# Healthcare-Robotics/assistive-vr-gym

Measured on AMD Instinct MI355X. Metric: env-steps/sec at N parallel envs, 1/2/4/8 MI355X; max |dq| vs PyBullet, higher is better.
Workload: dtype f32; 1 GPU; FeedingJaco-v0, 4096 envs/GPU, rigid-only, random actions; task=FeedingJaco-v0, envs_per_gpu=4096, impairment=random, parallelism=env-sharded x1, env_groups=4, stepping=rollout

## Files before the change

assistive-vr-gym_amd/csrc/avr_kernel.hip:

```cpp
#include <hip/hip_runtime.h>
#include <stdint.h>

#include "../../include/avr.h"
#include <cstring>
#include <cstdlib>
#include "avr_math.h"

#include "avr_kmodel.h"

typedef float f2v __attribute__((ext_vector_type(2)));
typedef float f4v __attribute__((ext_vector_type(4)));
typedef __attribute__((address_space(3))) float lds_f;
#define AVR_GA __attribute__((address_space(1)))
template <class T> __device__ __forceinline__ T gld(const T *p) { return *(const AVR_GA T *)p; }
__device__ __forceinline__ int2 gld(const int2 *p) { const AVR_GA int *q = (const AVR_GA int *)p; return make_int2(q[0], q[1]); }
__device__ __forceinline__ float2 gld(const float2 *p) { const f2v x = *(const AVR_GA f2v *)p; return make_float2(x.x, x.y); }
__device__ __forceinline__ float4 gld(const float4 *p) { const f4v x = *(const AVR_GA f4v *)p; return make_float4(x.x, x.y, x.z, x.w); }
__device__ __forceinline__ v3 gld3(const float *p) { const AVR_GA float *q = (const AVR_GA float *)p; return V(q[0], q[1], q[2]); }
__device__ __forceinline__ qt gldq(const float *p) { const AVR_GA float *q = (const AVR_GA float *)p; return Q(q[0], q[1], q[2], q[3]); }
__device__ __forceinline__ tf gldtf(const float *p) { tf r; r.p = gld3(p); r.q = gldq(p + 3); return r; }
typedef __attribute__((address_space(3))) f2v lds_f2;
typedef __attribute__((address_space(3))) f4v lds_f4;
typedef __attribute__((address_space(3))) int lds_i;
typedef const __attribute__((address_space(1))) float *gfp;
// ... 3380 lines not shown
        pcount(36, sm);
        pcount(37, mx);
        pcount(38, __popcll(__ballot(pk == 3)));
        pcount(39, __popcll(__ballot(pk >= 0 && pk < 3)));
#endif
    }
}

__global__ __launch_bounds__(64) __attribute__((amdgpu_waves_per_eu(NP_WAVES))) void avr_narrowphase_kernel(const KModel *__restrict__ mp, const float *__restrict__ state,
                                                             const unsigned char *__restrict__ mask, int env0, int n_envs) {
    const int list = (blockIdx.x >> 3) & 1;
    const int eb = env0 + 8 * NP_ENVS * (blockIdx.x >> 4) + (blockIdx.x & 7);
    if (eb >= n_envs) return;
    __shared__ float2 ent[NP_ENVS * MAXSP];
    __shared__ float btfs[NP_ENVS][MAXB * 8];
    __shared__ __attribute__((aligned(16))) int hkey[NP_HOT_KEYS];
    np_list(*mp, state, mask, eb, list, n_envs, ent, btfs, hkey);
}

#ifndef AVR_COOP_KERNEL
#define AVR_COOP_KERNEL 0
#endif
#if AVR_COOP_KERNEL
__global__ __launch_bounds__(64) void avr_coop_kernel(const KModel *__restrict__ mp, const unsigned char *__restrict__ mask, int env0, int n_envs) {
    __shared__ EpaBuf E;
    AVR_ENV_GUARD();
    if (gld(env_cs(m, env) + CS_COOP) != 0.f) {
        float *ws = env_ws(m, env);
        const int rot = __float_as_int(gld(ws + WS_COOPROT));
        (void)np_coop(m, env_cs(m, env), __float_as_int(gld(env_cs(m, env) + CS_NSP)), E, rot, 1 << 30);
        if (lane_id() == 0) ws[WS_COOPROT] = __int_as_float(rot + AVR_COOP_CAP);
    }
}
#endif

AVR_DI void substep_a_env(const KModel &m, EnvLDS &L, float *__restrict__ state, float dt, int env, int n_envs) {
    (void)n_envs;
    WT_START();
    static_assert(sizeof(EpaBuf) <= sizeof(EnvLDS), "EPA buffer overlay");
#if !AVR_COOP_KERNEL
    float *gst = state + (size_t)env * K_STATE_WORDS;
    const bool persist = gld(gst + S_TASK + T_COOPN) >= (float)AVR_COOP_PERSIST;
    int demand = 0;
    if (gld(env_cs(m, env) + CS_COOP) != 0.f) {
        float *ws = env_ws(m, env);
        const int rot = __float_as_int(gld(ws + WS_COOPROT));
        demand = np_coop(m, env_cs(m, env), __float_as_int(gld(env_cs(m, env) + CS_NSP)), *reinterpret_cast<EpaBuf *>(&L), rot,
                         persist ? AVR_COOP_CAP : 1 << 30);
        if (lane_id() == 0) ws[WS_COOPROT] = __int_as_float(rot + AVR_COOP_CAP);
        SYNC();
    }
#endif
#if AVR_COOP_KERNEL
    float *gst = state + (size_t)env * K_STATE_WORDS;
#endif
    load_a(m, L, gst, env_cs(m, env));
#if !AVR_COOP_KERNEL
    if (lane_id() == 0) {
        L.st[S_TASK + T_COOPN] = demand > AVR_COOP_CAP ? L.st[S_TASK + T_COOPN] + 1.f : 0.f;
        if (persist && demand > AVR_COOP_CAP) L.flags |= 32;
    }
    SYNC();
#endif
    bool ok = substep_a(m, L, dt, gst, env_ws(m, env), env_rows(m, env), env_cs(m, env), K_DYN_ROLE ? env_dynho(m, env) : nullptr);
#ifdef AVR_PROF
    if (lane_id() == 0) env_ws(m, env)[WS_XCC] = __int_as_float(xcc_id());
#endif
    if (lane_id() == 0 && !ok) L.flags |= 1;
    SYNC();
    if (lane_id() == 0) L.st[S_TASK + T_FLAGS] = (float)((int)L.st[S_TASK + T_FLAGS] | L.flags);
    SYNC();
    if (lane_id() < 16) gst[S_TASK + lane_id()] = L.st[S_TASK + lane_id()];
    prof_flush(m, L, env);
    WT_END(0);
}

__global__ __launch_bounds__(64) AVR_KATTR void avr_substep_a_kernel(const KModel *__restrict__ mp, float *__restrict__ state,
                                                                     const unsigned char *__restrict__ mask, float dt, int env0, int n_envs) {
    __shared__ EnvLDS L;
    AVR_ENV_GUARD();
    substep_a_env(m, L, state, dt, env, n_envs);
}

#if B4_PK
struct DV { float rq, rq2; f2v v1, v2, v3; };
#else
struct DV { float rq, rq2, vx, vy, vz, wx, wy, wz; };
#endif

AVR_DI int uni(int x) { return __builtin_amdgcn_readfirstlane(x); }

#define B4_OOB 0x7fff0000
typedef __amdgpu_buffer_rsrc_t rsrc_t;
typedef unsigned u4v __attribute__((ext_vector_type(4)));
typedef unsigned u3v __attribute__((ext_vector_type(3)));
typedef unsigned u2v __attribute__((ext_vector_type(2)));
AVR_DI f4v bld4(rsrc_t r, int o) { u4v x = __builtin_amdgcn_raw_buffer_load_b128(r, o, 0, 0); return *(f4v *)&x; }
AVR_DI f2v bld2(rsrc_t r, int o) { u2v x = __builtin_amdgcn_raw_buffer_load_b64(r, o, 0, 0); return *(f2v *)&x; }
AVR_DI float bld1(rsrc_t r, int o) { return __uint_as_float(__builtin_amdgcn_raw_buffer_load_b32(r, o, 0, 0)); }
#if NDL == 2
typedef f4v rv_t;
#define RVB 16
#define rload bld4
#else
typedef f2v rv_t;
#define RVB 8
#define rload bld2
#endif
typedef __attribute__((address_space(3))) rv_t lds_rv;
AVR_DI f4v bld3(rsrc_t r, int o) {
    u3v x = __builtin_amdgcn_raw_buffer_load_b96(r, o, 0, 0);
    f4v y = {__uint_as_float(x.x), __uint_as_float(x.y), __uint_as_float(x.z), 0.f};
    return y;
}

#ifndef B4_LDSW
#define B4_LDSW 10240
#endif
AVR_DI int al4(int x) { return (x + 3) & ~3; }

#ifndef B4_ADDR
#define B4_ADDR 1
#endif
#define B4_NP (B4_ADDR && B4_NC_LDS ? 1 : 0)
AVR_DI unsigned lds_addr(const __attribute__((address_space(3))) void *p) { return (unsigned)(size_t)p; }
AVR_DI __attribute__((address_space(3))) float *lds_at(unsigned a) { return (__attribute__((address_space(3))) float *)(size_t)a; }

AVR_DI int own_of(int mask) {
    const int sl = lane_id() & 15;
    return (int)__builtin_amdgcn_ubfe((unsigned)mask, sl < MAXF ? 2 * sl : 30, 2);
}
static_assert(2 * MAXF <= CI_SLOT && MAXNC + K_CROWS * K_MAX_CONTACTS < (1 << (30 - CI_SLOT)), "own mask and slot bit fields");


struct NcRow { int o; lds_f *ip; f4v h0, h1; float imp; f2v j0, j1, j2; rv_t r; };
struct NcSrc {
    typedef NcRow Row;
    static constexpr bool robot_parts = true, addr = false;
    rsrc_t rs;
    int eo, ro;
    lds_f *ip0, *nullip;
    AVR_DI void set(Row &R, bool v, int o, lds_f *ip) const { R.o = v ? o : B4_OOB; R.ip = v ? ip : nullip; }
    AVR_DI void hdr(Row &R) const { R.h0 = bld4(rs, R.o); R.h1 = bld3(rs, R.o + 16); R.imp = *R.ip; }
    AVR_DI void parts(Row &R) const {
        const int o = own_of(__float_as_int(R.h0.x));
        const int b = o ? R.o + 8 + 24 * o : B4_OOB;
        R.j0 = bld2(rs, b); R.j1 = bld2(rs, b + 8); R.j2 = bld2(rs, b + 16);
        const int slot = __float_as_int(R.h0.y) - 1;
        R.r = rload(rs, slot >= 0 ? ro + slot * (ROBW * 4) + RVB * (lane_id() & 15) : B4_OOB);
    }
};

#define LN_HEAD (NDL == 2 ? 80 : 48)
#define LNB_NULL 24
#define LNB_ZERO 48
#define LNB_NCNULL 16
typedef __attribute__((address_space(3))) char lds_c;
struct NcLds {
    typedef NcRow Row;
    static constexpr bool robot_parts = true, addr = B4_ADDR != 0;
    lds_c *blk;
    int eo;
    unsigned rob;
    lds_f *ip0, *nullip;
    AVR_DI void set(Row &R, bool v, int o, lds_f *ip) const { R.o = v ? o : LNB_NCNULL; R.ip = v ? ip : nullip; }
    AVR_DI void hdr(Row &R) const {
        R.h0 = *(const lds_f4 *)(blk + R.o - 8);
        const f2v a = *(const lds_f2 *)(blk + R.o + 8);
        R.h1.x = a.x; R.h1.y = a.y; R.h1.z = *(const lds_f *)(blk + R.o + 16);
        R.imp = *R.ip;
    }
    AVR_DI void parts(Row &R) const {
        const int w = own_of(__float_as_int(R.h0.x));
        const lds_f2 *q = (const lds_f2 *)(blk + (w ? R.o + 24 * w : LNB_ZERO));
        R.j0 = q[0]; R.j1 = q[1]; R.j2 = q[2];
        const unsigned sp = (unsigned)__float_as_int(R.h0.y);
        R.r = *(const lds_rv *)(blk + (sp ? rob + ROBW * 4 * sp : LNB_ZERO));
    }
};

struct CRowL { unsigned wb; lds_f *ip; f4v h; float imp; f2v j0, j1, j2; rv_t r; };
template <bool RC>
struct CLds {
    typedef CRowL Row;
    static constexpr bool robot_parts = RC, addr = B4_ADDR != 0;
    lds_c *blk;
    unsigned cn, cf;
    unsigned rob;
    lds_f *ipn, *ipf, *nullip;
    unsigned ct;
    lds_f *ipt;
    AVR_DI void set(Row &R, bool v, unsigned wb, lds_f *ip) const { R.wb = v ? wb : LNB_NULL; R.ip = v ? ip : nullip; }
    AVR_DI void hdr(Row &R) const { R.h = *(const lds_f4 *)(blk + R.wb + 8); R.imp = *R.ip; }
    AVR_DI void hdr3(Row &R) const {
        const lds_f *q = (const lds_f *)(blk + R.wb + 8);
        const f2v a = *(const lds_f2 *)q;
        R.h.x = a.x; R.h.y = a.y; R.h.z = q[2];
        R.imp = *R.ip;
    }
    AVR_DI void hdr2(Row &B, const Row &A) const {
        B.h = *(const lds_f4 *)(blk + A.wb + 8 + CRW * 4);
        B.imp = A.ip[1];
    }
    AVR_DI unsigned own_b(const Row &R) const { const int o = own_of(__float_as_int(R.h.x)); return o ? R.wb + 24 * o : LNB_ZERO; }
    AVR_DI void own_at(Row &R, unsigned b) const { const lds_f2 *q = (const lds_f2 *)(blk + b); R.j0 = q[0]; R.j1 = q[1]; R.j2 = q[2]; }
    AVR_DI unsigned rob_b(const Row &R) const { const unsigned s = (unsigned)__float_as_int(R.h.x) >> CI_SLOT; return s ? rob + ROBW * 4 * s : LNB_ZERO; }
    AVR_DI rv_t rob_at(unsigned b) const {
// ... 49 lines not shown
#pragma clang fp contract(off)
#if B4_PK
    f2v s = X.j0 * d.v1;
    if (RP) {
        s.y = fmaf(X.r.x, d.rq, s.y);
#if NDL == 2
        s.y = fmaf(X.r.z, d.rq2, s.y);
#endif
    }
    s = __builtin_elementwise_fma(X.j1, d.v2, s);
    s = __builtin_elementwise_fma(X.j2, d.v3, s);
    const float dv = row16_sum(s.x + s.y);
    const float ni = __builtin_amdgcn_fmed3f(imp + fmaf(-dv, inv, rhs), lo, hi);
    const float delta = ni - imp;
    if (acc) *acc |= __ballot(fabsf(delta) > rl);
    const f2v dd = {delta, delta};
    d.v1 = __builtin_elementwise_fma(X.j0, dd, d.v1);
    d.v2 = __builtin_elementwise_fma(X.j1, dd, d.v2);
    d.v3 = __builtin_elementwise_fma(X.j2, dd, d.v3);
    if (RP) d.rq = fmaf(X.r.y, delta, d.rq);
#if NDL == 2
    if (RP) d.rq2 = fmaf(X.r.w, delta, d.rq2);
#endif
    return ni;
#else
    const float p = fmaf(X.j1.x, d.vz, fmaf(X.j0.y, d.vy, X.j0.x * d.vx));
#if NDL == 2
    const float q = RP ? fmaf(X.j2.y, d.wz, fmaf(X.j2.x, d.wy, fmaf(X.r.z, d.rq2, fmaf(X.r.x, d.rq, X.j1.y * d.wx))))
                       : fmaf(X.j2.y, d.wz, fmaf(X.j2.x, d.wy, X.j1.y * d.wx));
#else
    const float q = RP ? fmaf(X.j2.y, d.wz, fmaf(X.j2.x, d.wy, fmaf(X.r.x, d.rq, X.j1.y * d.wx)))
                       : fmaf(X.j2.y, d.wz, fmaf(X.j2.x, d.wy, X.j1.y * d.wx));
#endif
    const float dv = row16_sum(p + q);
    const float ni = __builtin_amdgcn_fmed3f(imp + fmaf(-dv, inv, rhs), lo, hi);
    const float delta = ni - imp;
    if (acc) *acc |= __ballot(fabsf(delta) > rl);
    d.vx = fmaf(X.j0.x, delta, d.vx); d.vy = fmaf(X.j0.y, delta, d.vy); d.vz = fmaf(X.j1.x, delta, d.vz);
    d.wx = fmaf(X.j1.y, delta, d.wx); d.wy = fmaf(X.j2.x, delta, d.wy); d.wz = fmaf(X.j2.y, delta, d.wz);
    if (RP) d.rq = fmaf(X.r.y, delta, d.rq);
#if NDL == 2
    if (RP) d.rq2 = fmaf(X.r.w, delta, d.rq2);
#endif
    return ni;
#endif
}

#if B4_FPAIR
template <bool RP, class R>
AVR_DI void go4_pair(const R &A, const R &B, DV &d, float &ia, float &ib, float lim) {
#pragma clang fp contract(off)
    f2v sa = A.j0 * d.v1, sb = B.j0 * d.v1;
    if (RP) {
        sa.y = fmaf(A.r.x, d.rq, sa.y); sb.y = fmaf(B.r.x, d.rq, sb.y);
#if NDL == 2
        sa.y = fmaf(A.r.z, d.rq2, sa.y); sb.y = fmaf(B.r.z, d.rq2, sb.y);
#endif
    }
    sa = __builtin_elementwise_fma(A.j1, d.v2, sa); sb = __builtin_elementwise_fma(B.j1, d.v2, sb);
    sa = __builtin_elementwise_fma(A.j2, d.v3, sa); sb = __builtin_elementwise_fma(B.j2, d.v3, sb);
    const float dva = row16_sum(sa.x + sa.y), dvb0 = row16_sum(sb.x + sb.y);
    const float na = __builtin_amdgcn_fmed3f(ia + fmaf(-dva, A.h.y, A.h.z), -lim, lim);
    const float da = na - ia;
    const float dvb = fmaf(da, B.h.w, dvb0);
    const float nb = __builtin_amdgcn_fmed3f(ib + fmaf(-dvb, B.h.y, B.h.z), -lim, lim);
    const float db = nb - ib;
    const f2v dda = {da, da}, ddb = {db, db};
    d.v1 = __builtin_elementwise_fma(B.j0, ddb, __builtin_elementwise_fma(A.j0, dda, d.v1));
    d.v2 = __builtin_elementwise_fma(B.j1, ddb, __builtin_elementwise_fma(A.j1, dda, d.v2));
    d.v3 = __builtin_elementwise_fma(B.j2, ddb, __builtin_elementwise_fma(A.j2, dda, d.v3));
    if (RP) d.rq = fmaf(B.r.y, db, fmaf(A.r.y, da, d.rq));
#if NDL == 2
    if (RP) d.rq2 = fmaf(B.r.w, db, fmaf(A.r.w, da, d.rq2));
#endif
    ia = na; ib = nb;
}
#endif

template <int D, bool H3, class S>
AVR_DI void hdr_of(const S &s, typename S::Row &R) {
    if constexpr (H3) s.hdr3(R);
    else s.hdr(R);
}
template <int D, bool H3, class S, class AT, class GO>
AVR_DI void sweep4(const S &s, int n, const AT &at, const GO &go) {
    if (n <= 0) return;
    constexpr int K = 2 * D + 1;
    typename S::Row R[K];
#pragma unroll
    for (int q = 0; q < 2 * D; q++) { at(R[q], q); hdr_of<D, H3>(s, R[q]); }
#pragma unroll
    for (int q = 0; q < D; q++) s.parts(R[q]);
    for (int j = 0; j < n; j += K) {
#pragma unroll
        for (int q = 0; q < K; q++) {
            at(R[(q + 2 * D) % K], j + q + 2 * D);
            hdr_of<D, H3>(s, R[(q + 2 * D) % K]);
            s.parts(R[(q + D) % K]);
            go(R[q]);
        }
    }
}

template <class S>
struct Pair4 { typename S::Row a, b; float in; };

#if K_TORSION
template <class CS>
struct TorRow : CS::Row { float in; };
template <class CS>
struct TorSrc {
    typedef TorRow<CS> Row;
    static constexpr bool robot_parts = CS::robot_parts;
    const CS &cs;
    AVR_DI void hdr(Row &R) const { cs.hdr(R); }
    AVR_DI void parts(Row &R) const { cs.parts(R); }
};
#endif

AVR_DI int wave_max4(int x) {
    x = max(x, __shfl_xor(x, 16));
    x = max(x, __shfl_xor(x, 32));
    return uni(x);
}

template <int DN, int DC, class NS, class CS>
AVR_DI int pgs4(const KModel &m, const NS &ns, const CS &cs, lds_i *list, lds_i *tlist, int n_nc, int n_c, int nnc_max, int nc_max, DV &d) {
    typedef typename NS::Row NR;
    typedef typename CS::Row CR;
    const int sl = lane_id() & 15;
#if B4_PK
    d.rq = d.rq2 = 0.f; d.v1 = d.v2 = d.v3 = f2v{0.f, 0.f};
#else
    d.rq = d.rq2 = 0.f; d.vx = d.vy = d.vz = d.wx = d.wy = d.wz = 0.f;
#endif
    auto at_n = [&](CR &R, int j) {
        if constexpr (CS::addr) {
            const unsigned k = (unsigned)min(j, n_c);
            R.wb = cs.cn + CRW * 4 * k;
            R.ip = (lds_f *)((lds_c *)cs.ipn + __umul24(k, 12u));
        } else cs.set(R, j < n_c, cs.cn + CRW * 4 * j, cs.ipn + j);
    };
    sweep4<DC, true>(cs, nc_max, at_n, [&](const CR &R) { (void)go4<CS::robot_parts>(R, d, 0.f, R.h.y, R.h.z, R.imp, R.imp); });
    int units = 0;
    bool done = false;
    for (int it = 0; it < m.iters; it++) {
        const int a_nc = done ? 0 : n_nc, a_c = done ? 0 : n_c;
        const int anc_max = wave_max4(a_nc), ac_max = wave_max4(a_c);
        unsigned long long acc = 0ull;
        const bool fwd = (it & 1) != 0;
        const int r0 = fwd ? 0 : n_nc - 1, sg = fwd ? 1 : -1;
        const int ob = ns.eo + r0 * (RWC * 4);
        lds_f *ib = ns.ip0 + r0;
        const int no = fwd ? n_nc - a_nc : a_nc - 1;
        sweep4<DN, false>(ns, anc_max, [&](NR &R, int j) {
                              if constexpr (NS::addr) {
                                  const unsigned k = min((unsigned)(no + sg * j), (unsigned)n_nc);
                                  R.o = ns.eo + (int)__umul24(k, (unsigned)(RWC * 4));
                                  R.ip = ns.ip0 + k;
                              } else ns.set(R, j < a_nc, ob + sg * j * (RWC * 4), ib + sg * j);
                          },
                          [&](const NR &R) { *R.ip = go4<true>(R, d, R.imp, R.h0.z, R.h0.w, R.h1.x, R.h1.y, R.h1.z, &acc); });
        unsigned nb = cs.cn + CRW * 4 * (n_c - a_c);
        lds_c *const nib = (lds_c *)cs.ipn + 12 * (n_c - a_c);
        if constexpr (CS::addr) asm("" : "+v"(nb));
        auto at_na = [&](CR &R, int j) {
            if constexpr (CS::addr) {
                const unsigned k = (unsigned)min(j, a_c);
                R.wb = nb + CRW * 4 * k;
                R.ip = (lds_f *)(nib + __umul24(k, 12u));
            } else cs.set(R, j < a_c, cs.cn + CRW * 4 * j, cs.ipn + j);
        };
        sweep4<DC, false>(cs, ac_max, at_na, [&](const CR &R) { *R.ip = go4<CS::robot_parts>(R, d, R.imp, R.h.y, R.h.z, 0.f, 1e10f, R.h.w, &acc); });
        int t = 0;
        for (int c0 = 0; c0 < ac_max; c0 += 16) {
            const int c = c0 + sl;
            const bool a = c < a_c && cs.ipn[(CS::addr ? 3 : 1) * (c < a_c ? c : 0)] > 0.f;
            const unsigned long long b = __ballot(a);
            const unsigned gm = (unsigned)(b >> (lane_id() & 48)) & 0xffffu;
            if constexpr (CS::addr) {
                if (a) list[t + __popc(gm & ((1u << sl) - 1u))] = (int)((cs.cf + 2 * CRW * 4 * c) | lds_addr(cs.ipf + 3 * c) << 16);
            } else if (a) list[t + __popc(gm & ((1u << sl) - 1u))] = c;
            t += __popc(gm);
        }
        if constexpr (CS::addr) list[t] = (int)((unsigned)LNB_NULL | lds_addr(cs.nullip) << 16);
        const int tmax = wave_max4(t);
        units += tmax;
        if (tmax > 0) {
        constexpr int K = 2 * DC + 1;
        Pair4<CS> X[K];
        auto lst = [&](int u) {
            if constexpr (CS::addr) return list[min(u, t)];
            else { const int c = list[u < t ? u : 0]; return u < t ? c : -1; }
        };
        auto hdr = [&](Pair4<CS> &Y, int c) {
            if constexpr (CS::addr) {
                Y.a.wb = (unsigned)c & 0xffffu;
                Y.a.ip = lds_at((unsigned)c >> 16);
                cs.hdr(Y.a);
                cs.hdr2(Y.b, Y.a);
                Y.in = Y.a.ip[2];
            } else {
                cs.set(Y.a, c >= 0, cs.cf + 2 * CRW * 4 * c, cs.ipf + 2 * c);
                cs.hdr(Y.a);
                cs.hdr2(Y.b, Y.a);
                const float x = cs.ipn[max(c, 0)];
                Y.in = c >= 0 ? x : 0.f;
            }
        };
        auto go = [&](const Pair4<CS> &Y) {
            const float lim = Y.a.h.w * Y.in;
#if B4_FPAIR
            float ia = Y.a.imp, ib = Y.b.imp;
            go4_pair<CS::robot_parts>(Y.a, Y.b, d, ia, ib, lim);
            Y.a.ip[0] = ia; Y.a.ip[1] = ib;
#else
            Y.a.ip[0] = go4<CS::robot_parts>(Y.a, d, Y.a.imp, Y.a.h.y, Y.a.h.z, -lim, lim, Y.b.h.x, &acc);
            Y.a.ip[1] = go4<CS::robot_parts>(Y.b, d, Y.b.imp, Y.b.h.y, Y.b.h.z, -lim, lim, Y.b.h.w, &acc);
#endif
        };
        int cn = lst(0);
#pragma unroll
        for (int q = 0; q < 2 * DC; q++) { hdr(X[q], cn); cn = lst(q + 1); }
#pragma unroll
        for (int q = 0; q < DC; q++) cs.unit_parts(X[q].a, X[q].b);
        for (int u0 = 0; u0 < tmax; u0 += K) {
#pragma unroll
            for (int q = 0; q < K; q++) {
                hdr(X[(q + 2 * DC) % K], cn);
                cn = lst(u0 + q + 2 * DC + 1);
                cs.unit_parts(X[(q + DC) % K].a, X[(q + DC) % K].b);
                go(X[q]);
            }
        }
#if K_TORSION
        if constexpr (CS::addr) {
            typedef __attribute__((address_space(3))) u2v lds_u2;
            lds_u2 *const tl = (lds_u2 *)tlist;
            int tt = 0;
            for (int u0 = 0; u0 < tmax; u0 += 16) {
                const int u = u0 + sl;
                const unsigned e = (unsigned)list[min(u, t)];
                const int c = u < t ? (int)((e & 0xffffu) - cs.cf) >> 7 : 0;
                const int tv = cs.tor_of(c);
                const float in = lds_at(e >> 16)[2];
                const bool a = u < t && tv > 0;
                const unsigned long long b = __ballot(a);
                const unsigned gm = (unsigned)(b >> (lane_id() & 48)) & 0xffffu;
                if (a) {
                    lds_u2 *const q = tl + 3 * (tt + __popc(gm & ((1u << sl) - 1u)));
                    const unsigned w = (cs.ct + 3 * CRW * 4 * (tv - 1)) | lds_addr(cs.ipt + 3 * (tv - 1)) << 16;
#pragma unroll
                    for (int k = 0; k < 3; k++) q[k] = u2v{w + k * (CRW * 4 + (4 << 16)), (unsigned)__float_as_int(in)};
                }
                tt += __popc(gm);
            }
            const int tr = 3 * tt;
            tl[tr] = u2v{(unsigned)LNB_NULL | lds_addr(cs.nullip) << 16, 0u};
            const int ttmax = wave_max4(tt);
            const TorSrc<CS> ts{cs};
            sweep4<DC, false>(ts, 3 * ttmax, [&](TorRow<CS> &R, int j) {
                const u2v e = tl[min(j, tr)];
                R.wb = e.x & 0xffffu;
                R.ip = lds_at(e.x >> 16);
                R.in = __uint_as_float(e.y);
            }, [&](const TorRow<CS> &R) {
                const float lim = R.h.w * R.in;
                *R.ip = go4<CS::robot_parts>(R, d, R.imp, R.h.y, R.h.z, -lim, lim, BT_RESIDUAL_SQRT * R.h.y, &acc);
            });
        } else {
            int tt = 0;
            for (int u0 = 0; u0 < tmax; u0 += 16) {
                const int u = u0 + sl;
                const int cl = list[u < t ? u : 0];
                const int c = u < t ? cl : 0;
                const int tv = cs.tor_of(c);
                const bool a = u < t && tv > 0;
                const unsigned long long b = __ballot(a);
                const unsigned gm = (unsigned)(b >> (lane_id() & 48)) & 0xffffu;
                if (a) tlist[tt + __popc(gm & ((1u << sl) - 1u))] = c | (tv - 1) << 8;
                tt += __popc(gm);
            }
            int ttmax = tt;
            ttmax = max(ttmax, __shfl_xor(ttmax, 16));
            ttmax = max(ttmax, __shfl_xor(ttmax, 32));
            ttmax = uni(ttmax);
            const TorSrc<CS> ts{cs};
            sweep4<DC, false>(ts, 3 * ttmax, [&](TorRow<CS> &R, int j) {
                const int u = j / 3, k = j - 3 * u;
                const bool v = u < tt;
                const int e = tlist[v ? u : 0];
                const int c = e & 255, ti = e >> 8;
                cs.set(R, v, cs.ct + 3 * CRW * 4 * ti + CRW * 4 * k, cs.ipt + 3 * ti + k);
                const float x = cs.ipn[v ? c : 0];
                R.in = v ? x : 0.f;
            }, [&](const TorRow<CS> &R) {
                const float lim = R.h.w * R.in;
                *R.ip = go4<CS::robot_parts>(R, d, R.imp, R.h.y, R.h.z, -lim, lim, BT_RESIDUAL_SQRT * R.h.y, &acc);
            });
        }
#endif
        }
        done = done || ((acc >> (lane_id() & 48)) & 0xffffull) == 0ull;
        if (__ballot(!done) == 0ull) break;
    }
    return units;
}

#ifndef B4_DN
#define B4_DN 2
#endif
#ifndef B4_DC
#define B4_DC 1
#endif
#ifndef B4_DG
#define B4_DG 3
#endif
#ifndef B4_NC_LDS
#define B4_NC_LDS K_PR2
#endif
#ifndef B4_DNL
#define B4_DNL 1
#endif

#ifndef B4_SORT
#define B4_SORT 0
#endif
AVR_DI int b4_env(const KModel &m, const unsigned char *__restrict__ mask, int env0, int n_envs, int bidx, int g) {
    const int x = bidx & 7, j = bidx >> 3;
#if B4_SORT
    const int lane = lane_id();
    const int kc = (j >> 5) << 7;
    unsigned key[2];
#pragma unroll
    for (int h = 0; h < 2; h++) {
        const int kk = lane + 64 * h;
        const int e = env0 + x + 8 * (kc + kk);
        unsigned cost = 0xffffffu;
        if (e < n_envs) {
            cost = 0u;
            if (!mask || mask[e]) {
                const float *ws = env_ws(m, e);
                cost = (unsigned)(__float_as_int(gld(ws + WS_NNC)) + 3 * __float_as_int(gld(ws + WS_NC)) +
                                  (K_TORSION ? 3 * __float_as_int(gld(ws + WS_NT)) : 0));
                cost = min(cost, 0xfffffeu);
            }
        }
        key[h] = (cost << 7) | (unsigned)kk;
    }
    int rank0 = 0, rank1 = 0;
    for (int i = 0; i < 64; i++) {
        const unsigned a = __builtin_amdgcn_readlane(key[0], i), b = __builtin_amdgcn_readlane(key[1], i);
        rank0 += (a < key[0]) + (b < key[0]);
        rank1 += (a < key[1]) + (b < key[1]);
    }
    int pick = 0;
#pragma unroll
    for (int gg = 0; gg < 4; gg++) {
        const int r = 4 * (j & 31) + gg;
        const unsigned long long b0 = __ballot(rank0 == r), b1 = __ballot(rank1 == r);
        const int kk = b0 ? __builtin_ctzll(b0) : 64 + __builtin_ctzll(b1);
        if (g == gg) pick = kk;
    }
    return env0 + x + 8 * (kc + pick);
#else
    (void)m; (void)mask; (void)n_envs;
    return env0 + 32 * j + x + 8 * g;
#endif
}

AVR_DI void substep_b4_block(const KModel &m, float *__restrict__ state, const unsigned char *__restrict__ mask, float dt, int frame_end,
                             int env0, int n_envs, int bidx, lds_f *blk) {
#ifdef AVR_WAVETIME
    const unsigned long long wt0 = __builtin_amdgcn_s_memrealtime();
#endif
    const int lane = lane_id(), sl = lane & 15, g = lane >> 4;
    const int env = b4_env(m, mask, env0, n_envs, bidx, g);
    const bool live = env < n_envs && (!mask || mask[env]);
    const int ev = live ? env : env0;
    const gfp wsg = (gfp)env_ws(m, ev);
    float *st = state + (size_t)ev * K_STATE_WORDS;
    const int n_nc = live ? __float_as_int(wsg[WS_NNC]) : 0, n_c = live ? __float_as_int(wsg[WS_NC]) : 0;
    const int n_rob = live ? __float_as_int(wsg[WS_NROB]) : 0;
    const int n_t = live && K_TORSION ? __float_as_int(wsg[WS_NT]) : 0;
    const int n_cr = 3 * n_c + 3 * n_t;
    const int n_rows = n_nc + n_cr, n_rc = max(n_rob - n_nc, 0);
    auto wmax = [&](int x) { x = max(x, __shfl_xor(x, 16)); x = max(x, __shfl_xor(x, 32)); return uni(x); };
// ... 3 lines not shown
#ifdef AVR_LDS_POISON
    for (int i = lane; i < B4_LDSW; i += 64) blk[i] = __int_as_float(-1);
    SYNC();
#endif
#if B4_ADDR
    constexpr int GN = 4, GNC = 8;
    const int n_imp = n_rows + 3 + B4_NP;
    const int szA = al4(n_imp) + al4(n_c + 1) + (K_TORSION ? al4(6 * n_t + 2) : 0), szB = n_cr * CRW + n_rc * ROBW + GN;
#else
    constexpr int GN = 0, GNC = 0;
    const int n_imp = n_rows + 2;
    const int szA = al4(n_imp) + (K_TORSION ? 2 : 1) * al4(n_c), szB = n_cr * CRW + n_rc * ROBW;
#endif
#if B4_NC_LDS
    const int szF = szB + n_nc * (RWC + ROBW) + GNC;
    const int f0 = __shfl(szA + szF, 0), f1 = __shfl(szA + szF, 16), f2 = __shfl(szA + szF, 32), f3 = __shfl(szA + szF, 48);
    const bool full = uni(f0 + f1 + f2 + f3) <= B4_LDSW - LN_HEAD && !m.b4_global;
#else
    const int f0 = 0, f1 = 0, f2 = 0;
    constexpr bool full = false;
#endif
    const int t0 = __shfl(szA + szB, 0), t1 = __shfl(szA + szB, 16), t2 = __shfl(szA + szB, 32), t3 = __shfl(szA + szB, 48);
    const bool in_lds = full || (uni(t0 + t1 + t2 + t3) <= B4_LDSW - LN_HEAD && !m.b4_global);
    int base;
    if (full) base = g == 0 ? 0 : g == 1 ? f0 : g == 2 ? f0 + f1 : f0 + f1 + f2;
    else if (in_lds) base = g == 0 ? 0 : g == 1 ? t0 : g == 2 ? t0 + t1 : t0 + t1 + t2;
    else {
        const int a0 = __shfl(szA, 0), a1 = __shfl(szA, 16), a2 = __shfl(szA, 32);
        base = g == 0 ? 0 : g == 1 ? a0 : g == 2 ? a0 + a1 : a0 + a1 + a2;
    }
    base += LN_HEAD;
    lds_f *imp = blk + base;
    lds_i *list = (lds_i *)(imp + al4(n_imp));
    lds_i *tlist = list + al4(n_c + (B4_ADDR ? 1 : 0));
    const int cw = base + szA, nw = cw + n_cr * CRW + GN, rw = full ? nw + n_nc * RWC + GNC : nw;
    const bool trip = B4_ADDR && in_lds;
    const int ins = trip ? 3 : 1;
    lds_f *const ipt = trip ? imp + n_nc + B4_NP : imp + n_nc + 3 * n_c;
    lds_f *const ipf = trip ? ipt + 3 * n_t : imp + n_nc + n_c;
    lds_f *const ipn = trip ? ipf + 2 : imp + n_nc;
    lds_f *const nullip = trip ? ipf + 3 * n_c : imp + n_rows;
    const gfp cpool = (gfp)(st + S_CP);
    float wimp[K_MAX_CONTACTS / 16];
#pragma unroll
    for (int q = 0; q < K_MAX_CONTACTS / 16; q++) wimp[q] = cpool[AVR_CP_WORDS * min(sl + 16 * q, max(n_c - 1, 0)) + AVR_CP_IMP];
    for (int r = sl; r < n_imp; r += 16) {
        const int c = r - (int)(ipn - imp);
        if (!(c >= 0 && c < ins * n_c && (!trip || c % 3 == 0))) imp[r] = 0.f;
    }
    for (int i = lane; i < LN_HEAD; i += 64) blk[i] = 0.f;
    if (in_lds) {
        const int n4r = n_cr * (CRW / 4), n4n = full ? n_nc * (RWC / 4) : 0, n4s = (full ? n_rob : n_rc) * (ROBW / 4);
        const int n4a = n4r + n4n, n4 = n4a + n4s, so = full ? ro : ro + n_nc * ROBW * 4;
        const int m4 = wmax(n4);
        lds_f4 *l0 = (lds_f4 *)(blk + cw);
        for (int b = 0; b < m4; b += 8 * 16) {
            f4v t[8];
#pragma unroll
            for (int q = 0; q < 8; q++) {
                const int i = b + 16 * q + sl;
                t[q] = bld4(rs, i < n4r ? eo + CR_BASE * 4 + 16 * i : i < n4a ? eo + 16 * (i - n4r) : (i < n4 ? so + 16 * (i - n4a) : B4_OOB));
            }
#pragma unroll
            for (int q = 0; q < 8; q++) {
                const int i = b + 16 * q + sl;
#if B4_ADDR
                if (i < n4) l0[i + (i >= 4 * n_c ? GN / 4 : 0) + (full && i >= n4a ? GNC / 4 : 0)] = t[q];
#else
                if (i < n4) l0[i] = t[q];
#endif
            }
        }
#if B4_ADDR
        if (sl == 0) l0[4 * n_c] = f4v{0.f, 0.f, 0.f, 0.f};
        if (full && sl < GNC / 4) l0[n4a + GN / 4 + sl] = f4v{0.f, 0.f, 0.f, 0.f};
#endif
    }
#pragma unroll
    for (int q = 0; q < K_MAX_CONTACTS / 16; q++)
        if (sl + 16 * q < n_c) ipn[ins * (sl + 16 * q)] = wimp[q] * m.warmstart;
    SYNC();
    NcSrc ns{rs, eo, ro, imp, nullip};
    DV d;
    int units, rcb = 0;
#if B4_NC_LDS
    if (full) {
        const unsigned cn = 4 * cw - 8, cf = cn + 4 * CRW * n_c + 4 * GN, ct = cf + 8 * CRW * n_c, rob = 4 * (rw - ROBW) + RVB * sl;
        const NcLds nl{(lds_c *)blk, 4 * nw + 8, rob, imp, nullip};
        if (wmax(n_rc) > 0) {
            CLds<true> cs{(lds_c *)blk, cn, cf, rob, ipn, ipf, nullip, ct, ipt};
            units = pgs4<B4_DNL, B4_DC>(m, nl, cs, list, tlist, n_nc, n_c, nnc_max, nc_max, d);
            rcb = 1;
        } else {
            CLds<false> cs{(lds_c *)blk, cn, cf, rob, ipn, ipf, nullip, ct, ipt};
            units = pgs4<B4_DNL, B4_DC>(m, nl, cs, list, tlist, n_nc, n_c, nnc_max, nc_max, d);
        }
    } else
#endif
    if (in_lds) {
        const unsigned cn = 4 * cw - 8, cf = cn + 4 * CRW * n_c + 4 * GN, ct = cf + 8 * CRW * n_c, rob = 4 * (rw - (n_nc + 1) * ROBW) + RVB * sl;
        if (wmax(n_rc) > 0) {
            CLds<true> cs{(lds_c *)blk, cn, cf, rob, ipn, ipf, nullip, ct, ipt};
            units = pgs4<B4_DN, B4_DC>(m, ns, cs, list, tlist, n_nc, n_c, nnc_max, nc_max, d);
            rcb = 1;
        } else {
            CLds<false> cs{(lds_c *)blk, cn, cf, rob, ipn, ipf, nullip, ct, ipt};
            units = pgs4<B4_DN, B4_DC>(m, ns, cs, list, tlist, n_nc, n_c, nnc_max, nc_max, d);
        }
    } else {
        const int cn = eo + CR_BASE * 4, cf = cn + 4 * CRW * n_c, ct = cf + 8 * CRW * n_c, rob = ro - ROBW * 4 + RVB * sl;
        CGlb cs{rs, cn, cf, rob, ipn, ipf, nullip, ct, ipt};
        units = pgs4<B4_DN, B4_DG>(m, ns, cs, list, tlist, n_nc, n_c, nnc_max, nc_max, d);
    }
    (void)units; (void)rcb;
    for (int c = sl; c < n_c; c += 16) st[S_CP + AVR_CP_WORDS * c + AVR_CP_IMP] = ipn[ins * c];
#ifdef AVR_WAVETIME
    {
        const unsigned long long wt1 = __builtin_amdgcn_s_memrealtime();
        const int e0 = env0 + 32 * (bidx >> 3) + (bidx & 7);
        if (m.prof && lane == 0 && e0 < n_envs) {
            m.prof[((size_t)1 * n_envs + e0) * 2] = wt0;
            m.prof[((size_t)1 * n_envs + e0) * 2 + 1] = wt1;
            m.prof[((size_t)2 * n_envs + e0) * 2] = (unsigned long long)nnc_max | (unsigned long long)nc_max << 16 | (unsigned long long)in_lds << 32;
            m.prof[((size_t)2 * n_envs + e0) * 2 + 1] = (unsigned long long)wmax(n_rows) | (unsigned long long)units << 16 | (unsigned long long)rcb << 40 | (unsigned long long)xcc_id() << 44;
        }
    }
#endif
    if (!live) return;
    const float *ws = env_ws(m, ev);
#if B4_PK
    struct { float vx, vy, vz, wx, wy, wz; } dl = {d.v1.x, d.v2.x, d.v3.x, d.v1.y, d.v2.y, d.v3.y};
#else
    DV &dl = d;
#endif
    if (sl < m.nf) {
        const qt q = ldq(st + S_FREE + AVR_FB_WORDS * sl + 3);
        const v3 I = gld3(m.fb_inertia + 4 * sl);
        const float rs = 1.f / sqrtf(gld(m.fb_mass + (sl)));
        const v3 sd = V(sqrtf(I.x > 0.f ? 1.f / I.x : 0.f), sqrtf(I.y > 0.f ? 1.f / I.y : 0.f), sqrtf(I.z > 0.f ? 1.f / I.z : 0.f));
        const v3 w = qrot(q, V(dl.wx * sd.x, dl.wy * sd.y, dl.wz * sd.z));
        dl.vx *= rs; dl.vy *= rs; dl.vz *= rs;
        dl.wx = w.x; dl.wy = w.y; dl.wz = w.z;
    }
    const float vmax = m.max_vel;
    const int nda = env_hdyn(m, st) ? m.nd + m.hc_n : m.nd;
#pragma unroll
    for (int k = 0; k < NDL; k++) {
        const int dof = sl + 16 * k;
        if (dof < nda) {
            float v = clampf(ws[WS_VQ + dof] + (k == 0 ? d.rq : d.rq2), -vmax, vmax);
            float q = st[S_Q + dof] + dt * v;
            if (frame_end && dof >= m.nd) {
#if K_CHAIN_LIMITS_IN_STATE
                const float lo = st[S_HCH + 2 * K_HC_N + (dof - m.nd)], hi = st[S_HCH + 3 * K_HC_N + (dof - m.nd)];
#else
                const float lo = gld(m.hc_lower + (dof - m.nd)), hi = gld(m.hc_upper + (dof - m.nd));
#endif
                if (q < lo) { q = lo; v = 0.f; }
                else if (q > hi) { q = hi; v = 0.f; }
            }
            st[S_QD + dof] = v;
            st[S_Q + dof] = q;
        }
    }
    if (sl < m.nf) {
        float *fb = st + S_FREE + AVR_FB_WORDS * sl;
        v3 v = clamp3(add(ld3(ws + WS_FV + 4 * sl), V(dl.vx, dl.vy, dl.vz)), vmax);
        v3 om = clamp3(add(ld3(ws + WS_FW + 4 * sl), V(dl.wx, dl.wy, dl.wz)), vmax);
        st3(fb + 7, v);
        st3(fb + 10, om);
        st3(fb, add(ld3(fb), scl(v, dt)));
        float ang = len(om);
        if (ang * dt > BT_ANGULAR_MOTION_THRESHOLD) ang = (0.5f * 1.5707963267948966f) / dt;
        v3 ax;
        if (ang < 0.001f) ax = scl(om, 0.5f * dt - (dt * dt * dt) * 0.020833333333f * ang * ang);
        else ax = scl(om, sinf(0.5f * ang * dt) / ang);
        qt dq = Q(ax.x, ax.y, ax.z, cosf(ang * dt * 0.5f));
        stq(fb + 3, qnorm(qmul(dq, ldq(fb + 3))));
    }
}

__global__ __launch_bounds__(64) void avr_substep_b4_kernel(const KModel *__restrict__ mp, float *__restrict__ state,
                                                            const unsigned char *__restrict__ mask, float dt, int frame_end, int env0,
                                                            int n_envs) {
    __shared__ f4v b4l[B4_LDSW / 4];
    substep_b4_block(*mp, state, mask, dt, frame_end, env0, n_envs, blockIdx.x, (lds_f *)(lds_f4 *)b4l);
}



#if AVR_TASK == AVR_TASK_FEEDING
__global__ __launch_bounds__(64) void avr_task_kernel(const KModel *__restrict__ mp, float *__restrict__ state, float *__restrict__ obs,
                                                      float *__restrict__ rew, unsigned char *__restrict__ done, float *__restrict__ info,
                                                      const unsigned char *__restrict__ mask, int mode, int env0, int n_envs) {
    __shared__ EnvLDS L;
    AVR_ENV_GUARD();
    const int lane = lane_id();
    float *gst = state + (size_t)env * K_STATE_WORDS;
    const float *gcp = gst + S_CP;
    load_state(m, L, gst);
    PROF_START(ptask);
    if (L.nla > m.nl) robot_fk(m, L);
    mouth_target(m, L);
    if (mode == MODE_SETTLE) {
        if (obs) observe(m, L, 0.f, obs + (size_t)env * K_OBS_DIM);
    } else if (mode == MODE_STEP || mode == MODE_STEP_RANDOM) {
        if (lane == 0) L.st[S_TASK + T_ITER] += 1.f;
// ... 291 lines not shown
```

assistive-vr-gym_amd/csrc/avr_task.h:

```cpp
#pragma once
#include "../../include/avr_model.h"

#ifndef AVR_TASK
#error "AVR_TASK must be defined (AVR_TASK_FEEDING, AVR_TASK_SCRATCH or AVR_TASK_BEDBATH)"
#endif

#define T_TARGET 0
#define T_ITER 3
#define T_SUCCESS 4
#define T_GENDER 7
#define T_FLAGS 8
#define T_NCP 9
#define T_HDYN 10
#define T_COOPN 15

#if AVR_TASK == AVR_TASK_FEEDING
#define K_MAX_LINKS AVR_MAX_LINKS
#define K_MAX_DOF AVR_MAX_DOF
#define K_HC_N AVR_HC_N
#define K_MAX_FREE AVR_MAX_FREE
#define K_MAX_HUMAN AVR_MAX_HUMAN
#define K_MAX_CONTACTS AVR_MAX_CONTACTS
#define K_ACT_DIM AVR_ACT_DIM
#define K_OBS_DIM AVR_OBS_DIM
#define S_Q AVR_S_Q
#define S_QD AVR_S_QD
#define S_QTGT AVR_S_QTGT
#define S_KP AVR_S_KP
#define S_MAXIMP AVR_S_MAXIMP
#define S_FREE AVR_S_FREE
#define S_TASK AVR_S_TASK
#define S_HUMAN AVR_S_HUMAN
#define S_HCH AVR_S_HCH
#define S_CP AVR_S_CP
#define K_STATE_WORDS AVR_STATE_WORDS
#define K_T_WORDS AVR_T_WORDS
#define T_ALIVE AVR_T_ALIVE
#define T_HIT AVR_T_HIT
#define K_RBASE_IN_STATE 0
#define K_CHAIN_LIMITS_IN_STATE 0
#define K_HUMAN_GRAVITY 0
#define K_TOOL_PIVOT 0
#define K_PR2 0
#define K_ND 10
#define K_TORSION 0
#define K_DYN_ROLE 1
#define K_PAIRS_FLAT 1
#define K_NP_HOT 1
#elif AVR_TASK == AVR_TASK_SCRATCH || AVR_TASK == AVR_TASK_BEDBATH
#define K_PR2 1
#define K_ND 14
#define K_DYN_ROLE 0
#define K_PAIRS_FLAT 1
#define K_NP_HOT 0
#define K_MAX_LINKS AVR_SI_MAX_LINKS
#define K_MAX_DOF AVR_SI_MAX_DOF
#define K_HC_N AVR_SI_HC_N
#define K_MAX_FREE AVR_SI_MAX_FREE
#define K_MAX_HUMAN AVR_SI_MAX_HUMAN
#define K_MAX_CONTACTS AVR_SI_MAX_CONTACTS
#define K_ACT_DIM AVR_SI_ACT_DIM
#if AVR_TASK == AVR_TASK_BEDBATH
#define K_OBS_DIM AVR_BB_OBS_DIM
#define T_WIPE AVR_BB_T_WIPE
#define T_NTGT AVR_BB_T_NTGT
#else
#define K_OBS_DIM AVR_SI_OBS_DIM
#endif
#define S_Q AVR_SI_S_Q
#define S_QD AVR_SI_S_QD
#define S_QTGT AVR_SI_S_QTGT
#define S_KP AVR_SI_S_KP
#define S_MAXIMP AVR_SI_S_MAXIMP
#define S_FREE AVR_SI_S_FREE
#define S_RBASE AVR_SI_S_RBASE
#define S_TASK AVR_SI_S_TASK
#define S_HUMAN AVR_SI_S_HUMAN
#define S_HCH AVR_SI_S_HCH
#define S_CP AVR_SI_S_CP
#define K_STATE_WORDS AVR_SI_STATE_WORDS
#define K_T_WORDS AVR_SI_T_WORDS
#define T_LIMB AVR_SI_T_LIMB
#define T_STRENGTH AVR_SI_T_STRENGTH
#define T_PREV AVR_SI_T_PREV
#define T_TREMOR AVR_SI_T_TREMOR
#define T_ONARM AVR_SI_T_ONARM
#define K_RBASE_IN_STATE 1
#define K_CHAIN_LIMITS_IN_STATE 1
#define K_HUMAN_GRAVITY 1
#define K_TOOL_PIVOT 1
#define K_TORSION 1
#else
#error "unknown AVR_TASK"
#endif
#define K_CROWS (K_TORSION ? 6 : 3)
```

Measured before the change: 979,600 env-steps/s.

## Prefetch next PGS iteration's non-contact row headers during contact sweep and batch contact list

Splits sweep4 into header, parts and rounds phases so the non-contact row headers and parts for the next PGS iteration can be issued ahead of time, during the contact sweep and list build of the current iteration. This hides load latency at iteration boundaries. It also restructures the active-contact list compaction to preload all impulses before the ballots. It is enabled for the feeding task only, and adds register pressure plus a re-prime step whenever a lane's done state changes. Optional wave timestamps are added under AVR_WAVETIME.

```diff
diff --git a/assistive-vr-gym_amd/csrc/avr_kernel.hip b/assistive-vr-gym_amd/csrc/avr_kernel.hip
--- a/assistive-vr-gym_amd/csrc/avr_kernel.hip
+++ b/assistive-vr-gym_amd/csrc/avr_kernel.hip
@@ -3486,10 +3486,17 @@
     substep_a_env(m, L, state, dt, env, n_envs);
 }
 
+#ifdef AVR_WAVETIME
+#define WT_FIELDS unsigned long long wt_stage, wt_warm, wt_it0, wt_epi;
+#define WT_STAMP(x) do { __builtin_amdgcn_sched_barrier(0); (x) = __builtin_amdgcn_s_memrealtime(); __builtin_amdgcn_sched_barrier(0); } while (0)
+#else
+#define WT_FIELDS
+#define WT_STAMP(x) do { } while (0)
+#endif
 #if B4_PK
-struct DV { float rq, rq2; f2v v1, v2, v3; };
+struct DV { float rq, rq2; f2v v1, v2, v3; WT_FIELDS };
 #else
-struct DV { float rq, rq2, vx, vy, vz, wx, wy, wz; };
+struct DV { float rq, rq2, vx, vy, vz, wx, wy, wz; WT_FIELDS };
 #endif
 
 AVR_DI int uni(int x) { return __builtin_amdgcn_readfirstlane(x); }
@@ -3527,6 +3534,15 @@
 #define B4_ADDR 1
 #endif
 #define B4_NP (B4_ADDR && B4_NC_LDS ? 1 : 0)
+#ifndef B4_FIXED
+#define B4_FIXED K_B4_FIXED
+#endif
+#ifndef B4_FX_LIST
+#define B4_FX_LIST B4_FIXED
+#endif
+#ifndef B4_FX_AHEAD
+#define B4_FX_AHEAD B4_FIXED
+#endif
 AVR_DI unsigned lds_addr(const __attribute__((address_space(3))) void *p) { return (unsigned)(size_t)p; }
 AVR_DI __attribute__((address_space(3))) float *lds_at(unsigned a) { return (__attribute__((address_space(3))) float *)(size_t)a; }
 
@@ -3742,15 +3758,19 @@
     if constexpr (H3) s.hdr3(R);
     else s.hdr(R);
 }
+template <int D, bool H3, class S, class AT>
+AVR_DI void sweep4_hdrs(const S &s, typename S::Row (&R)[2 * D + 1], const AT &at) {
+#pragma unroll
+    for (int q = 0; q < 2 * D; q++) { at(R[q], q); hdr_of<D, H3>(s, R[q]); }
+}
+template <int D, class S>
+AVR_DI void sweep4_parts(const S &s, typename S::Row (&R)[2 * D + 1]) {
+#pragma unroll
+    for (int q = 0; q < D; q++) s.parts(R[q]);
+}
 template <int D, bool H3, class S, class AT, class GO>
-AVR_DI void sweep4(const S &s, int n, const AT &at, const GO &go) {
-    if (n <= 0) return;
+AVR_DI void sweep4_rounds(const S &s, int n, typename S::Row (&R)[2 * D + 1], const AT &at, const GO &go) {
     constexpr int K = 2 * D + 1;
-    typename S::Row R[K];
-#pragma unroll
-    for (int q = 0; q < 2 * D; q++) { at(R[q], q); hdr_of<D, H3>(s, R[q]); }
-#pragma unroll
-    for (int q = 0; q < D; q++) s.parts(R[q]);
     for (int j = 0; j < n; j += K) {
 #pragma unroll
         for (int q = 0; q < K; q++) {
@@ -3760,6 +3780,14 @@
             go(R[q]);
         }
     }
+}
+template <int D, bool H3, class S, class AT, class GO>
+AVR_DI void sweep4(const S &s, int n, const AT &at, const GO &go) {
+    if (n <= 0) return;
+    typename S::Row R[2 * D + 1];
+    sweep4_hdrs<D, H3>(s, R, at);
+    sweep4_parts<D>(s, R);
+    sweep4_rounds<D, H3>(s, n, R, at, go);
 }
 
 template <class S>
@@ -3802,25 +3830,39 @@
         } else cs.set(R, j < n_c, cs.cn + CRW * 4 * j, cs.ipn + j);
     };
     sweep4<DC, true>(cs, nc_max, at_n, [&](const CR &R) { (void)go4<CS::robot_parts>(R, d, 0.f, R.h.y, R.h.z, R.imp, R.imp); });
+    WT_STAMP(d.wt_warm);
+#ifdef AVR_WAVETIME
+    d.wt_it0 = d.wt_warm;
+#endif
     int units = 0;
     bool done = false;
+    auto nc_at = [&](int it_, int a) {
+        const bool fwd = (it_ & 1) != 0;
+        const int r0 = fwd ? 0 : n_nc - 1, sg = fwd ? 1 : -1;
+        const int ob = ns.eo + r0 * (RWC * 4);
+        lds_f *const ib = ns.ip0 + r0;
+        const int no = fwd ? n_nc - a : a - 1;
+        return [=, &ns](NR &R, int j) {
+            if constexpr (NS::addr) {
+                const unsigned k = min((unsigned)(no + sg * j), (unsigned)n_nc);
+                R.o = ns.eo + (int)__umul24(k, (unsigned)(RWC * 4));
+                R.ip = ns.ip0 + k;
+            } else ns.set(R, j < a, ob + sg * j * (RWC * 4), ib + sg * j);
+        };
+    };
+    constexpr bool AHEAD = B4_FX_AHEAD && CS::addr && !NS::addr;
+    NR Rn[2 * DN + 1];
+    if constexpr (AHEAD) {
+        sweep4_hdrs<DN, false>(ns, Rn, nc_at(0, n_nc));
+        sweep4_parts<DN>(ns, Rn);
+    }
     for (int it = 0; it < m.iters; it++) {
         const int a_nc = done ? 0 : n_nc, a_c = done ? 0 : n_c;
         const int anc_max = wave_max4(a_nc), ac_max = wave_max4(a_c);
         unsigned long long acc = 0ull;
-        const bool fwd = (it & 1) != 0;
-        const int r0 = fwd ? 0 : n_nc - 1, sg = fwd ? 1 : -1;
-        const int ob = ns.eo + r0 * (RWC * 4);
-        lds_f *ib = ns.ip0 + r0;
-        const int no = fwd ? n_nc - a_nc : a_nc - 1;
-        sweep4<DN, false>(ns, anc_max, [&](NR &R, int j) {
-                              if constexpr (NS::addr) {
-                                  const unsigned k = min((unsigned)(no + sg * j), (unsigned)n_nc);
-                                  R.o = ns.eo + (int)__umul24(k, (unsigned)(RWC * 4));
-                                  R.ip = ns.ip0 + k;
-                              } else ns.set(R, j < a_nc, ob + sg * j * (RWC * 4), ib + sg * j);
-                          },
-                          [&](const NR &R) { *R.ip = go4<true>(R, d, R.imp, R.h0.z, R.h0.w, R.h1.x, R.h1.y, R.h1.z, &acc); });
+        const auto go_nc = [&](const NR &R) { *R.ip = go4<true>(R, d, R.imp, R.h0.z, R.h0.w, R.h1.x, R.h1.y, R.h1.z, &acc); };
+        if constexpr (AHEAD) sweep4_rounds<DN, false>(ns, anc_max, Rn, nc_at(it, a_nc), go_nc);
+        else sweep4<DN, false>(ns, anc_max, nc_at(it, a_nc), go_nc);
         unsigned nb = cs.cn + CRW * 4 * (n_c - a_c);
         lds_c *const nib = (lds_c *)cs.ipn + 12 * (n_c - a_c);
         if constexpr (CS::addr) asm("" : "+v"(nb));
@@ -3832,7 +3874,25 @@
             } else cs.set(R, j < a_c, cs.cn + CRW * 4 * j, cs.ipn + j);
         };
         sweep4<DC, false>(cs, ac_max, at_na, [&](const CR &R) { *R.ip = go4<CS::robot_parts>(R, d, R.imp, R.h.y, R.h.z, 0.f, 1e10f, R.h.w, &acc); });
+        if constexpr (AHEAD) sweep4_hdrs<DN, false>(ns, Rn, nc_at(it + 1, a_nc));
         int t = 0;
+        if constexpr (B4_FX_LIST && CS::addr) {
+            constexpr int NR = (K_MAX_CONTACTS + 15) / 16;
+            float in[NR];
+#pragma unroll
+            for (int q = 0; q < NR; q++) { const int c = 16 * q + sl; in[q] = cs.ipn[3 * (c < a_c ? c : 0)]; }
+#pragma unroll
+            for (int q = 0; q < NR; q++) {
+                if (16 * q < ac_max) {
+                    const int c = 16 * q + sl;
+                    const bool a = c < a_c && in[q] > 0.f;
+                    const unsigned long long b = __ballot(a);
+                    const unsigned gm = (unsigned)(b >> (lane_id() & 48)) & 0xffffu;
+                    if (a) list[t + __popc(gm & ((1u << sl) - 1u))] = (int)((cs.cf + 2 * CRW * 4 * c) | lds_addr(cs.ipf + 3 * c) << 16);
+                    t += __popc(gm);
+                }
+            }
+        } else
         for (int c0 = 0; c0 < ac_max; c0 += 16) {
             const int c = c0 + sl;
             const bool a = c < a_c && cs.ipn[(CS::addr ? 3 : 1) * (c < a_c ? c : 0)] > 0.f;
@@ -3846,6 +3906,7 @@
         if constexpr (CS::addr) list[t] = (int)((unsigned)LNB_NULL | lds_addr(cs.nullip) << 16);
         const int tmax = wave_max4(t);
         units += tmax;
+        if constexpr (AHEAD) sweep4_parts<DN>(ns, Rn);
         if (tmax > 0) {
         constexpr int K = 2 * DC + 1;
         Pair4<CS> X[K];
@@ -3961,8 +4022,18 @@
         }
 #endif
         }
+        const bool was = done;
         done = done || ((acc >> (lane_id() & 48)) & 0xffffull) == 0ull;
+#ifdef AVR_WAVETIME
+        if (it == 0) WT_STAMP(d.wt_it0);
+#endif
         if (__ballot(!done) == 0ull) break;
+        if constexpr (AHEAD) {
+            if (__ballot(done != was) != 0ull) {
+                sweep4_hdrs<DN, false>(ns, Rn, nc_at(it + 1, done ? 0 : n_nc));
+                sweep4_parts<DN>(ns, Rn);
+            }
+        }
     }
     return units;
 }
@@ -4132,6 +4203,7 @@
     SYNC();
     NcSrc ns{rs, eo, ro, imp, nullip};
     DV d;
+    WT_STAMP(d.wt_stage);
     int units, rcb = 0;
 #if B4_NC_LDS
     if (full) {
@@ -4163,6 +4235,7 @@
         units = pgs4<B4_DN, B4_DG>(m, ns, cs, list, tlist, n_nc, n_c, nnc_max, nc_max, d);
     }
     (void)units; (void)rcb;
+    WT_STAMP(d.wt_epi);
     for (int c = sl; c < n_c; c += 16) st[S_CP + AVR_CP_WORDS * c + AVR_CP_IMP] = ipn[ins * c];
 #ifdef AVR_WAVETIME
     {
@@ -4173,6 +4246,12 @@
             m.prof[((size_t)1 * n_envs + e0) * 2 + 1] = wt1;
             m.prof[((size_t)2 * n_envs + e0) * 2] = (unsigned long long)nnc_max | (unsigned long long)nc_max << 16 | (unsigned long long)in_lds << 32;
             m.prof[((size_t)2 * n_envs + e0) * 2 + 1] = (unsigned long long)wmax(n_rows) | (unsigned long long)units << 16 | (unsigned long long)rcb << 40 | (unsigned long long)xcc_id() << 44;
+            if (e0 + 16 < n_envs) {
+                m.prof[((size_t)1 * n_envs + e0 + 8) * 2] = d.wt_stage;
+                m.prof[((size_t)1 * n_envs + e0 + 8) * 2 + 1] = d.wt_warm;
+                m.prof[((size_t)1 * n_envs + e0 + 16) * 2] = d.wt_it0;
+                m.prof[((size_t)1 * n_envs + e0 + 16) * 2 + 1] = d.wt_epi;
+            }
         }
     }
 #endif
diff --git a/assistive-vr-gym_amd/csrc/avr_task.h b/assistive-vr-gym_amd/csrc/avr_task.h
--- a/assistive-vr-gym_amd/csrc/avr_task.h
+++ b/assistive-vr-gym_amd/csrc/avr_task.h
@@ -47,12 +47,14 @@
 #define K_DYN_ROLE 1
 #define K_PAIRS_FLAT 1
 #define K_NP_HOT 1
+#define K_B4_FIXED 1
 #elif AVR_TASK == AVR_TASK_SCRATCH || AVR_TASK == AVR_TASK_BEDBATH
 #define K_PR2 1
 #define K_ND 14
 #define K_DYN_ROLE 0
 #define K_PAIRS_FLAT 1
 #define K_NP_HOT 0
+#define K_B4_FIXED 0
 #define K_MAX_LINKS AVR_SI_MAX_LINKS
 #define K_MAX_DOF AVR_SI_MAX_DOF
 #define K_HC_N AVR_SI_HC_N
```

New measurement: 990,300 env-steps/s (median of 6 runs). 1.1% higher.
